# lambdaclass/lambda_elliptic_curves

Hardware: AMD Instinct MI355X
Metric: NTT elems/sec (Stark252 radix-2, 2^24, forward, bit-exact vs CPU: see 'bit_exact') [+ MSM G1 point-adds/sec under 'msm'] (higher is better)
Workload: dtype u32x8 (256-bit Montgomery, 32-bit limbs)

## Files before the change

### lambda_elliptic_curves_amd/csrc/field.cuh

```cuda
#pragma once
#include <stdint.h>

#if defined(__HIPCC__)
#include <hip/hip_runtime.h>
#define LW_HD __host__ __device__ __forceinline__
#else
#define LW_HD inline
#endif

namespace lw {

struct Stark252 {
    static constexpr int N = 8;
    static constexpr bool LAZY = true;
    static constexpr uint32_t INV = 0xffffffffu;
    static constexpr uint32_t TWO_ADICITY = 192;
    LW_HD static constexpr uint32_t p(int i) {
        constexpr uint32_t t[N] = {0x00000001u, 0x00000000u, 0x00000000u, 0x00000000u, 0x00000000u, 0x00000000u, 0x00000011u, 0x08000000u};
        return t[i];
    }
    LW_HD static constexpr uint32_t one(int i) {
        constexpr uint32_t t[N] = {0xffffffe1u, 0xffffffffu, 0xffffffffu, 0xffffffffu, 0xffffffffu, 0xffffffffu, 0xfffffdf0u, 0x07ffffffu};
        return t[i];
    }
// ... 231 lines not shown
#pragma unroll
    for (int i = 0; i < N; i++) {
        uint64_t c = 0;
#pragma unroll
        for (int j = 0; j < N; j++) {
            c += (uint64_t)a.v[j] * b.v[i] + t[j];
            t[j] = (uint32_t)c;
            c >>= 32;
        }
        uint32_t tN = (uint32_t)c;
        uint32_t m = t[0] * F::INV;
        c = ((uint64_t)m * F::p(0) + t[0]) >> 32;
#pragma unroll
        for (int j = 1; j < N; j++) {
            c += (uint64_t)m * F::p(j) + t[j];
            t[j - 1] = (uint32_t)c;
            c >>= 32;
        }
        c += tN;
        t[N - 1] = (uint32_t)c;
    }
    Fe<F> r;
#pragma unroll
    for (int i = 0; i < N; i++) r.v[i] = t[i];
    return reduce_once<F>(r);
}

#if !defined(__HIP_DEVICE_COMPILE__) && defined(__SIZEOF_INT128__)
#define LW_HOST_MUL64 1
template <class F>
inline Fe<F> fe_mul_host64(const Fe<F> &a, const Fe<F> &b) {
    constexpr int N = F::N, M = N / 2;
    static_assert(N % 2 == 0, "even number of 32-bit limbs");
    typedef unsigned __int128 u128;
    uint64_t A[M], B[M], P[M], t[M + 2];
    for (int i = 0; i < M; i++) {
        A[i] = (uint64_t)a.v[2 * i] | ((uint64_t)a.v[2 * i + 1] << 32);
        B[i] = (uint64_t)b.v[2 * i] | ((uint64_t)b.v[2 * i + 1] << 32);
        P[i] = (uint64_t)F::p(2 * i) | ((uint64_t)F::p(2 * i + 1) << 32);
    }
    for (int i = 0; i < M + 2; i++) t[i] = 0;
    uint64_t z = (uint64_t)(0u - F::INV);
    z *= 2 - P[0] * z;
    const uint64_t inv = 0 - z;
    for (int i = 0; i < M; i++) {
        u128 c = 0;
        for (int j = 0; j < M; j++) {
            c += (u128)A[j] * B[i] + t[j];
            t[j] = (uint64_t)c;
            c >>= 64;
        }
        c += t[M];
        t[M] = (uint64_t)c;
        t[M + 1] = (uint64_t)(c >> 64);
        const uint64_t m = t[0] * inv;
        c = ((u128)m * P[0] + t[0]) >> 64;
        for (int j = 1; j < M; j++) {
            c += (u128)m * P[j] + t[j];
            t[j - 1] = (uint64_t)c;
            c >>= 64;
        }
        c += t[M];
        t[M - 1] = (uint64_t)c;
        t[M] = t[M + 1] + (uint64_t)(c >> 64);
    }
    Fe<F> r;
    for (int i = 0; i < M; i++) {
        r.v[2 * i] = (uint32_t)t[i];
        r.v[2 * i + 1] = (uint32_t)(t[i] >> 32);
    }
    return reduce_once<F>(r);
}
#endif

#if defined(__HIP_DEVICE_COMPILE__)
#define LW_MAC_V(A, B) "v_mad_u64_u32 %0, vcc, " A ", " B ", %0\n\tv_addc_co_u32_e32 %1, vcc, 0, %1, vcc\n\t"

__device__ __forceinline__ void mac96_x1(uint64_t &lo, uint32_t &hi, uint32_t a0, uint32_t b0) {
    asm(LW_MAC_V("%2", "%3") : "+v"(lo), "+v"(hi) : "v"(a0), "v"(b0) : "vcc");
}
__device__ __forceinline__ void mac96_x2(uint64_t &lo, uint32_t &hi, uint32_t a0, uint32_t b0, uint32_t a1, uint32_t b1) {
    asm(LW_MAC_V("%2", "%3") LW_MAC_V("%4", "%5") : "+v"(lo), "+v"(hi) : "v"(a0), "v"(b0), "v"(a1), "v"(b1) : "vcc");
}
__device__ __forceinline__ void mac96_x4(uint64_t &lo, uint32_t &hi, uint32_t a0, uint32_t b0, uint32_t a1, uint32_t b1,
                                         uint32_t a2, uint32_t b2, uint32_t a3, uint32_t b3) {
    asm(LW_MAC_V("%2", "%3") LW_MAC_V("%4", "%5") LW_MAC_V("%6", "%7") LW_MAC_V("%8", "%9")
        : "+v"(lo), "+v"(hi)
        : "v"(a0), "v"(b0), "v"(a1), "v"(b1), "v"(a2), "v"(b2), "v"(a3), "v"(b3)
        : "vcc");
}
#define LW_MAC_FIRST(A, B, INIT) "v_mad_u64_u32 %0, vcc, " A ", " B ", " INIT "\n\tv_addc_co_u32_e64 %1, vcc, 0, 0, vcc\n\t"
__device__ __forceinline__ void mac96_first_x1(uint64_t &lo, uint32_t &hi, uint64_t init, uint32_t a0, uint32_t b0) {
    asm(LW_MAC_FIRST("%3", "%4", "%2") : "=v"(lo), "=v"(hi) : "v"(init), "v"(a0), "v"(b0) : "vcc");
}
__device__ __forceinline__ void mac96_first_x2(uint64_t &lo, uint32_t &hi, uint64_t init, uint32_t a0, uint32_t b0, uint32_t a1,
                                               uint32_t b1) {
    asm(LW_MAC_FIRST("%3", "%4", "%2") LW_MAC_V("%5", "%6")
        : "=&v"(lo), "=&v"(hi) : "v"(init), "v"(a0), "v"(b0), "v"(a1), "v"(b1) : "vcc");
}
__device__ __forceinline__ void mac96_first_x4(uint64_t &lo, uint32_t &hi, uint64_t init, uint32_t a0, uint32_t b0, uint32_t a1,
                                               uint32_t b1, uint32_t a2, uint32_t b2, uint32_t a3, uint32_t b3) {
    asm(LW_MAC_FIRST("%3", "%4", "%2") LW_MAC_V("%5", "%6") LW_MAC_V("%7", "%8") LW_MAC_V("%9", "%10")
        : "=&v"(lo), "=&v"(hi)
        : "v"(init), "v"(a0), "v"(b0), "v"(a1), "v"(b1), "v"(a2), "v"(b2), "v"(a3), "v"(b3)
        : "vcc");
}
template <uint32_t C>
__device__ __forceinline__ void mac96_c1(uint64_t &lo, uint32_t &hi, uint32_t m0) {
    if constexpr (C == 0) {
    } else if constexpr (C <= 64) {
        asm(LW_MAC_V("%2", "%3") : "+v"(lo), "+v"(hi) : "v"(m0), "n"(C) : "vcc");
    } else {
        asm(LW_MAC_V("%2", "%3") : "+v"(lo), "+v"(hi) : "v"(m0), "s"(C) : "vcc");
    }
}
template <uint32_t C0, uint32_t C1, uint32_t C2, uint32_t C3>
__device__ __forceinline__ void mac96_s4(uint64_t &lo, uint32_t &hi, uint32_t m0, uint32_t m1, uint32_t m2, uint32_t m3) {
    asm(LW_MAC_V("%2", "%3") LW_MAC_V("%4", "%5") LW_MAC_V("%6", "%7") LW_MAC_V("%8", "%9")
        : "+v"(lo), "+v"(hi)
        : "v"(m0), "s"(C0), "v"(m1), "s"(C1), "v"(m2), "s"(C2), "v"(m3), "s"(C3)
        : "vcc");
}

template <class F, int K, int I, int IEND>
__device__ __forceinline__ void col_ab(uint64_t &lo, uint32_t &hi, const Fe<F> &a, const Fe<F> &b) {
    if constexpr (I + 4 <= IEND) {
        mac96_x4(lo, hi, a.v[I], b.v[K - I], a.v[I + 1], b.v[K - I - 1], a.v[I + 2], b.v[K - I - 2], a.v[I + 3], b.v[K - I - 3]);
        col_ab<F, K, I + 4, IEND>(lo, hi, a, b);
    } else if constexpr (I + 2 <= IEND) {
        mac96_x2(lo, hi, a.v[I], b.v[K - I], a.v[I + 1], b.v[K - I - 1]);
        col_ab<F, K, I + 2, IEND>(lo, hi, a, b);
    } else if constexpr (I + 1 <= IEND) {
        mac96_x1(lo, hi, a.v[I], b.v[K - I]);
    }
}
template <uint32_t C>
constexpr bool lw_is_literal() { return C > 64; }
template <class F, int K, int I, int IEND>
__device__ __forceinline__ void col_mp(uint64_t &lo, uint32_t &hi, const uint32_t (&m)[F::N]) {
    if constexpr (I + 4 <= IEND) {
        if constexpr (lw_is_literal<F::p(K - I)>() && lw_is_literal<F::p(K - I - 1)>() && lw_is_literal<F::p(K - I - 2)>() &&
                      lw_is_literal<F::p(K - I - 3)>()) {
            mac96_s4<F::p(K - I), F::p(K - I - 1), F::p(K - I - 2), F::p(K - I - 3)>(lo, hi, m[I], m[I + 1], m[I + 2], m[I + 3]);
            col_mp<F, K, I + 4, IEND>(lo, hi, m);
        } else {
            mac96_c1<F::p(K - I)>(lo, hi, m[I]);
            col_mp<F, K, I + 1, IEND>(lo, hi, m);
        }
    } else if constexpr (I + 1 <= IEND) {
        mac96_c1<F::p(K - I)>(lo, hi, m[I]);
        col_mp<F, K, I + 1, IEND>(lo, hi, m);
    }
}
#include "mac_chains.inc"

template <class F, int LO, int HI>
constexpr bool lw_all_literal() {
    for (int i = LO; i < HI; i++)
        if (F::p(i) <= 64) return false;
    return true;
}

template <class F, int K, int I, int IEND>
__device__ __forceinline__ void col_ab_first(uint64_t &lo, uint32_t &hi, uint64_t init, const Fe<F> &a, const Fe<F> &b) {
    if constexpr (I + 4 <= IEND) {
        mac96_first_x4(lo, hi, init, a.v[I], b.v[K - I], a.v[I + 1], b.v[K - I - 1], a.v[I + 2], b.v[K - I - 2], a.v[I + 3], b.v[K - I - 3]);
        col_ab<F, K, I + 4, IEND>(lo, hi, a, b);
    } else if constexpr (I + 2 <= IEND) {
        mac96_first_x2(lo, hi, init, a.v[I], b.v[K - I], a.v[I + 1], b.v[K - I - 1]);
        col_ab<F, K, I + 2, IEND>(lo, hi, a, b);
    } else {
        static_assert(I + 1 <= IEND, "column without products");
        mac96_first_x1(lo, hi, init, a.v[I], b.v[K - I]);
    }
}
template <class F, int P, int K>
__device__ __forceinline__ void fips_col(uint64_t init, const Fe<F> *const (&a)[P], const Fe<F> *const (&b)[P], uint32_t (&m)[F::N],
                                         uint32_t (&t)[F::N]) {
    constexpr int N = F::N;
    if constexpr (K == 2 * N - 1) {
        t[N - 1] = (uint32_t)init;
    } else {
        uint64_t lo;
        uint32_t hi;
        if constexpr (K < N) {
#if defined(LW_NO_COLUMN_CHAINS)
            col_ab_first<F, K, 0, K + 1>(lo, hi, init, *a[0], *b[0]);
#else
            col_ab_first_dispatch<F, K, 0, K + 1>(lo, hi, init, *a[0], *b[0]);
#endif
            if constexpr (P > 1) col_ab<F, K, 0, K + 1>(lo, hi, *a[1], *b[1]);
            if constexpr (P > 2) col_ab<F, K, 0, K + 1>(lo, hi, *a[2], *b[2]);
            if constexpr (P > 3) col_ab<F, K, 0, K + 1>(lo, hi, *a[3], *b[3]);
#if defined(LW_NO_COLUMN_CHAINS)
            col_mp<F, K, 0, K>(lo, hi, m);
#else
            if constexpr (K >= 1 && lw_all_literal<F, 1, K + 1>()) col_mp_dispatch<F, K, 0, K>(lo, hi, m);
            else col_mp<F, K, 0, K>(lo, hi, m);
#endif
            uint32_t mk;
            if constexpr (F::INV == 0xffffffffu) mk = 0u - (uint32_t)lo;
            else mk = (uint32_t)lo * F::INV;
            m[K] = mk;
            mac96_c1<F::p(0)>(lo, hi, mk);
        } else {
#if defined(LW_NO_COLUMN_CHAINS)
            col_ab_first<F, K, K - N + 1, N>(lo, hi, init, *a[0], *b[0]);
#else
            col_ab_first_dispatch<F, K, K - N + 1, 2 * N - 1 - K>(lo, hi, init, *a[0], *b[0]);
#endif
            if constexpr (P > 1) col_ab<F, K, K - N + 1, N>(lo, hi, *a[1], *b[1]);
            if constexpr (P > 2) col_ab<F, K, K - N + 1, N>(lo, hi, *a[2], *b[2]);
            if constexpr (P > 3) col_ab<F, K, K - N + 1, N>(lo, hi, *a[3], *b[3]);
#if defined(LW_NO_COLUMN_CHAINS)
            col_mp<F, K, K - N + 1, N>(lo, hi, m);
#else
            if constexpr (lw_all_literal<F, K - N + 1, N>()) col_mp_dispatch<F, K, K - N + 1, 2 * N - 1 - K>(lo, hi, m);
            else col_mp<F, K, K - N + 1, N>(lo, hi, m);
#endif
            t[K - N] = (uint32_t)lo;
        }
        fips_col<F, P, K + 1>((lo >> 32) | ((uint64_t)hi << 32), a, b, m, t);
    }
}
template <class F>
__device__ __forceinline__ Fe<F> fe_mul_gfx9(const Fe<F> &a, const Fe<F> &b) {
    constexpr int N = F::N;
    uint32_t m[N], t[N];
    const Fe<F> *const pa[1] = {&a}, *const pb[1] = {&b};
    fips_col<F, 1, 0>(0ull, pa, pb, m, t);
    Fe<F> r;
#pragma unroll
    for (int i = 0; i < N; i++) r.v[i] = t[i];
    return reduce_once<F>(r);
}
#endif

template <class F>
LW_HD Fe<F> fe_mul(const Fe<F> &a, const Fe<F> &b) {
#if defined(__HIP_DEVICE_COMPILE__)
    return fe_mul_gfx9<F>(a, b);
#elif defined(LW_HOST_MUL64)
    return fe_mul_host64<F>(a, b);
#else
    return fe_mul_portable<F>(a, b);
#endif
}

template <class F>
LW_HD Fe<F> fe_sqr(const Fe<F> &a) { return fe_mul<F>(a, a); }

template <class F>
LW_HD Fe<F> fe_neg_raw(const Fe<F> &a) {
    uint32_t pk[F::N];
    limbs_kp<F, 0>(pk);
    Fe<F> r;
    limbs_sub<F::N>(r.v, pk, a.v);
    return r;
}
template <class F>
LW_HD Fe<F> fe_neg_raw_2p(const Fe<F> &a) {
    uint32_t pk[F::N];
    limbs_kp<F, 1>(pk);
    Fe<F> r;
    limbs_sub<F::N>(r.v, pk, a.v);
    return r;
}
template <class F, int P, int KSUM = P>
LW_HD Fe<F> fe_dot(const Fe<F> *const (&a)[P], const Fe<F> *const (&b)[P]) {
    static_assert(P >= 1 && P <= 4, "fe_dot: 1..4 products");
    static_assert(KSUM >= P, "fe_dot: KSUM counts every product at least once");
    static_assert((uint64_t)KSUM * ((uint64_t)F::p(F::N - 1) + 1) <= (1ull << 32), "fe_dot: sum of products would exceed 2p after reduction");
#if defined(__HIP_DEVICE_COMPILE__)
    constexpr int N = F::N;
    uint32_t m[N], t[N];
    fips_col<F, P, 0>(0ull, a, b, m, t);
    Fe<F> r;
#pragma unroll
    for (int i = 0; i < N; i++) r.v[i] = t[i];
    return reduce_once<F>(r);
#else
    static_assert(KSUM == P, "fe_dot: unreduced operands are a device-code feature");
    Fe<F> acc = fe_mul<F>(reduce_once<F>(*a[0]), *b[0]);
    for (int q = 1; q < P; q++) acc = fe_add<F>(acc, fe_mul<F>(reduce_once<F>(*a[q]), *b[q]));
    return acc;
#endif
}

template <class F, int LOGK>
LW_HD Fe<F> fe_cond_sub_kp(const Fe<F> &a) {
    constexpr int N = F::N;
    uint32_t kp[N];
    limbs_kp<F, LOGK>(kp);
    Fe<F> d;
    const uint32_t borrow = limbs_sub<N>(d.v, a.v, kp);
    Fe<F> r;
#pragma unroll
    for (int i = 0; i < N; i++) r.v[i] = borrow ? a.v[i] : d.v[i];
    return r;
}
LW_HD Fe<Stark252> fe_reduce_full(const Fe<Stark252> &x) {
    const uint32_t q = x.v[7] >> 27;
    const uint32_t z = lw_k(0u);
    const uint32_t sub[8] = {q, z, z, z, z, z, 17u * q, q << 27};
    Fe<Stark252> d;
    const uint32_t borrow = limbs_sub<8>(d.v, x.v, sub);
    uint32_t pm[8];
    limbs_p_masked<Stark252>(pm, 0u - borrow);
    Fe<Stark252> r;
    limbs_add<8>(r.v, d.v, pm);
    return r;
}
template <class F>
LW_HD Fe<F> fe_reduce_full(const Fe<F> &x) { return reduce_once<F>(x); }

template <class F>
LW_HD Fe<F> fe_add_raw(const Fe<F> &a, const Fe<F> &b) {
    Fe<F> s;
    limbs_add<F::N>(s.v, a.v, b.v);
    return s;
}
template <class F>
LW_HD Fe<F> fe_add2p_sub_raw(const Fe<F> &a, const Fe<F> &b) {
    constexpr int N = F::N;
    uint32_t kp[N];
    limbs_kp<F, 1>(kp);
    Fe<F> d, r;
    limbs_sub<N>(d.v, a.v, b.v);
    limbs_add<N>(r.v, d.v, kp);
    return r;
}
template <class F>
LW_HD Fe<F> fe_mul_lazy(const Fe<F> &a, const Fe<F> &b) {
#if defined(__HIP_DEVICE_COMPILE__)
    constexpr int N = F::N;
    uint32_t m[N], t[N];
    const Fe<F> *const pa[1] = {&a}, *const pb[1] = {&b};
    fips_col<F, 1, 0>(0ull, pa, pb, m, t);
    Fe<F> r;
#pragma unroll
    for (int i = 0; i < N; i++) r.v[i] = t[i];
    return r;
#else
    return fe_mul_portable<F>(a, b);
#endif
}

template <class F>
LW_HD Fe<F> fe_pow_u64(Fe<F> base, uint64_t e) {
    Fe<F> r = Fe<F>::one();
    while (e) {
        if (e & 1) r = fe_mul<F>(r, base);
        base = fe_sqr<F>(base);
        e >>= 1;
    }
    return r;
}

template <class F>
LW_HD Fe<F> fe_inv(const Fe<F> &a) {
    constexpr int N = F::N;
    uint32_t e[N];
    uint64_t borrow = 2;
#pragma unroll
    for (int i = 0; i < N; i++) {
        uint64_t t = (uint64_t)F::p(i) - borrow;
        e[i] = (uint32_t)t;
        borrow = (t >> 32) & 1;
    }
    Fe<F> r = Fe<F>::one();
    for (int i = N - 1; i >= 0; i--) {
        for (int bit = 31; bit >= 0; bit--) {
            r = fe_sqr<F>(r);
            if ((e[i] >> bit) & 1) r = fe_mul<F>(r, a);
        }
    }
    return r;
}

template <class F>
LW_HD constexpr int fe_modulus_bits() {
    int top = 0;
    for (int b = 0; b < 32; b++)
        if ((F::p(F::N - 1) >> b) & 1u) top = b + 1;
    return 32 * (F::N - 1) + top;
}
template <int N>
LW_HD uint32_t bingcd_update_ab(uint32_t (&x)[N], uint32_t (&y)[N], int32_t f, int32_t g, int32_t h, int32_t k) {
    int64_t cx = 0, cy = 0;
    uint32_t wx[N + 1], wy[N + 1];
#pragma unroll
    for (int i = 0; i < N; i++) {
        const int64_t zx = (int64_t)x[i] * f + (int64_t)y[i] * g + cx;
        const int64_t zy = (int64_t)x[i] * h + (int64_t)y[i] * k + cy;
        wx[i] = (uint32_t)zx;
        wy[i] = (uint32_t)zy;
        cx = zx >> 32;
        cy = zy >> 32;
    }
    wx[N] = (uint32_t)cx;
    wy[N] = (uint32_t)cy;
    const uint32_t nx = (uint32_t)((uint64_t)cx >> 63), ny = (uint32_t)((uint64_t)cy >> 63);
    uint32_t carx = nx, cary = ny;
#pragma unroll
    for (int i = 0; i < N; i++) {
        uint32_t rx = (wx[i] >> 30) | (wx[i + 1] << 2), ry = (wy[i] >> 30) | (wy[i + 1] << 2);
        rx ^= 0u - nx;
        ry ^= 0u - ny;
        const uint32_t sx = rx + carx, sy = ry + cary;
        carx = sx < rx ? 1u : 0u;
        cary = sy < ry ? 1u : 0u;
        x[i] = sx;
        y[i] = sy;
    }
    return nx | (ny << 1);
}
template <class F>
LW_HD void bingcd_update_uv(uint32_t (&u)[F::N], uint32_t (&v)[F::N], int32_t f, int32_t g, int32_t h, int32_t k) {
    constexpr int N = F::N;
    const uint32_t fu = ((uint32_t)(u[0] * (uint32_t)f + v[0] * (uint32_t)g) * F::INV) & 0x3fffffffu;
    const uint32_t fv = ((uint32_t)(u[0] * (uint32_t)h + v[0] * (uint32_t)k) * F::INV) & 0x3fffffffu;
    int64_t cu = 0, cv = 0;
    uint32_t wu[N + 1], wv[N + 1];
#pragma unroll
    for (int i = 0; i < N; i++) {
        const int64_t zu = (int64_t)u[i] * f + (int64_t)v[i] * g + (int64_t)((uint64_t)F::p(i) * fu) + cu;
        const int64_t zv = (int64_t)u[i] * h + (int64_t)v[i] * k + (int64_t)((uint64_t)F::p(i) * fv) + cv;
        wu[i] = (uint32_t)zu;
        wv[i] = (uint32_t)zv;
        cu = zu >> 32;
        cv = zv >> 32;
    }
    wu[N] = (uint32_t)cu;
    wv[N] = (uint32_t)cv;
    const uint32_t nu = (uint32_t)((uint64_t)cu >> 63), nv = (uint32_t)((uint64_t)cv >> 63);
    uint32_t ru[N], rv[N];
#pragma unroll
    for (int i = 0; i < N; i++) {
        ru[i] = (wu[i] >> 30) | (wu[i + 1] << 2);
        rv[i] = (wv[i] >> 30) | (wv[i + 1] << 2);
    }
    uint32_t pk[N], du[N], dv[N], su[N], sv[N];
#pragma unroll
    for (int i = 0; i < N; i++) pk[i] = F::p(i);
    const uint32_t bu = limbs_sub<N>(du, ru, pk), bv = limbs_sub<N>(dv, rv, pk);
    limbs_add<N>(su, ru, pk);
    limbs_add<N>(sv, rv, pk);
#pragma unroll
    for (int i = 0; i < N; i++) {
        u[i] = nu ? su[i] : (bu ? ru[i] : du[i]);
        v[i] = nv ? sv[i] : (bv ? rv[i] : dv[i]);
    }
}
template <class F>
LW_HD Fe<F> fe_inv_int_bingcd(const Fe<F> &y) {
    constexpr int N = F::N;
    constexpr int ROUNDS = (2 * fe_modulus_bits<F>()) / 29 + 2;
    uint32_t a[N], b[N], u[N], v[N];
#pragma unroll
    for (int i = 0; i < N; i++) {
        a[i] = y.v[i];
        b[i] = F::p(i);
        u[i] = i == 0 ? 1u : 0u;
        v[i] = 0u;
    }
#pragma nounroll
    for (int round = 0; round < ROUNDS; round++) {
        uint32_t a0 = 0, a1 = 0, b0 = 0, b1 = 0, c0 = 0xffffffffu, c1 = 0xffffffffu;
#pragma unroll
        for (int j = N - 1; j >= 0; j--) {
            const uint32_t aw = a[j], bw = b[j];
            a0 ^= (a0 ^ aw) & c0;
            a1 ^= (a1 ^ aw) & c1;
            b0 ^= (b0 ^ bw) & c0;
            b1 ^= (b1 ^ bw) & c1;
            c1 = c0;
            c0 &= ((aw | bw) == 0u) ? 0xffffffffu : 0u;
        }
        a1 |= a0 & c1;
        a0 &= ~c1;
        b1 |= b0 & c1;
        b0 &= ~c1;
        uint64_t a_hi = ((uint64_t)a0 << 32) | a1, b_hi = ((uint64_t)b0 << 32) | b1;
        uint32_t a_lo = a[0], b_lo = b[0];
        int32_t pa = 1, pb = 0, qa = 0, qb = 1;
#pragma unroll 2
        for (int i = 0; i < 30; i++) {
            const uint32_t r = a_hi > b_hi ? 1u : 0u;
            const uint32_t oa = (a_lo >> i) & 1u, ob = (b_lo >> i) & 1u;
            const uint32_t cAB = oa & ob & r, cBA = oa & ob & (r ^ 1u), cA = cAB | (oa ^ 1u);
            const uint32_t mAB = 0u - cAB, mBA = 0u - cBA, mA = 0u - cA;
// ... 118 lines not shown
```

### lambda_elliptic_curves_amd/csrc/mac_chains.inc

```

template <class F, int K, int I>
__device__ __forceinline__ void col_ab_first_n1(uint64_t &lo, uint32_t &hi, uint64_t init, const Fe<F> &a, const Fe<F> &b) {
    asm(LW_MAC_FIRST("%3", "%4", "%2")
        : "=v"(lo), "=v"(hi)
        : "v"(init), "v"(a.v[I + 0]), "v"(b.v[K - I - 0])
        : "vcc");
}

template <class F, int K, int I>
__device__ __forceinline__ void col_ab_first_n2(uint64_t &lo, uint32_t &hi, uint64_t init, const Fe<F> &a, const Fe<F> &b) {
    asm(LW_MAC_FIRST("%3", "%4", "%2") LW_MAC_V("%5", "%6")
        : "=&v"(lo), "=&v"(hi)
        : "v"(init), "v"(a.v[I + 0]), "v"(b.v[K - I - 0]), "v"(a.v[I + 1]), "v"(b.v[K - I - 1])
        : "vcc");
}

template <class F, int K, int I>
__device__ __forceinline__ void col_ab_first_n3(uint64_t &lo, uint32_t &hi, uint64_t init, const Fe<F> &a, const Fe<F> &b) {
    asm(LW_MAC_FIRST("%3", "%4", "%2") LW_MAC_V("%5", "%6") LW_MAC_V("%7", "%8")
        : "=&v"(lo), "=&v"(hi)
        : "v"(init), "v"(a.v[I + 0]), "v"(b.v[K - I - 0]), "v"(a.v[I + 1]), "v"(b.v[K - I - 1]), "v"(a.v[I + 2]), "v"(b.v[K - I - 2])
        : "vcc");
}

// ... 39 lines not shown

template <class F, int K, int I>
__device__ __forceinline__ void col_ab_first_n9(uint64_t &lo, uint32_t &hi, uint64_t init, const Fe<F> &a, const Fe<F> &b) {
    asm(LW_MAC_FIRST("%3", "%4", "%2") LW_MAC_V("%5", "%6") LW_MAC_V("%7", "%8") LW_MAC_V("%9", "%10") LW_MAC_V("%11", "%12") LW_MAC_V("%13", "%14") LW_MAC_V("%15", "%16") LW_MAC_V("%17", "%18") LW_MAC_V("%19", "%20")
        : "=&v"(lo), "=&v"(hi)
        : "v"(init), "v"(a.v[I + 0]), "v"(b.v[K - I - 0]), "v"(a.v[I + 1]), "v"(b.v[K - I - 1]), "v"(a.v[I + 2]), "v"(b.v[K - I - 2]), "v"(a.v[I + 3]), "v"(b.v[K - I - 3]), "v"(a.v[I + 4]), "v"(b.v[K - I - 4]), "v"(a.v[I + 5]), "v"(b.v[K - I - 5]), "v"(a.v[I + 6]), "v"(b.v[K - I - 6]), "v"(a.v[I + 7]), "v"(b.v[K - I - 7]), "v"(a.v[I + 8]), "v"(b.v[K - I - 8])
        : "vcc");
}

template <class F, int K, int I>
__device__ __forceinline__ void col_ab_first_n10(uint64_t &lo, uint32_t &hi, uint64_t init, const Fe<F> &a, const Fe<F> &b) {
    asm(LW_MAC_FIRST("%3", "%4", "%2") LW_MAC_V("%5", "%6") LW_MAC_V("%7", "%8") LW_MAC_V("%9", "%10") LW_MAC_V("%11", "%12") LW_MAC_V("%13", "%14") LW_MAC_V("%15", "%16") LW_MAC_V("%17", "%18") LW_MAC_V("%19", "%20") LW_MAC_V("%21", "%22")
        : "=&v"(lo), "=&v"(hi)
        : "v"(init), "v"(a.v[I + 0]), "v"(b.v[K - I - 0]), "v"(a.v[I + 1]), "v"(b.v[K - I - 1]), "v"(a.v[I + 2]), "v"(b.v[K - I - 2]), "v"(a.v[I + 3]), "v"(b.v[K - I - 3]), "v"(a.v[I + 4]), "v"(b.v[K - I - 4]), "v"(a.v[I + 5]), "v"(b.v[K - I - 5]), "v"(a.v[I + 6]), "v"(b.v[K - I - 6]), "v"(a.v[I + 7]), "v"(b.v[K - I - 7]), "v"(a.v[I + 8]), "v"(b.v[K - I - 8]), "v"(a.v[I + 9]), "v"(b.v[K - I - 9])
        : "vcc");
}

template <class F, int K, int I>
__device__ __forceinline__ void col_ab_first_n11(uint64_t &lo, uint32_t &hi, uint64_t init, const Fe<F> &a, const Fe<F> &b) {
    asm(LW_MAC_FIRST("%3", "%4", "%2") LW_MAC_V("%5", "%6") LW_MAC_V("%7", "%8") LW_MAC_V("%9", "%10") LW_MAC_V("%11", "%12") LW_MAC_V("%13", "%14") LW_MAC_V("%15", "%16") LW_MAC_V("%17", "%18") LW_MAC_V("%19", "%20") LW_MAC_V("%21", "%22") LW_MAC_V("%23", "%24")
        : "=&v"(lo), "=&v"(hi)
        : "v"(init), "v"(a.v[I + 0]), "v"(b.v[K - I - 0]), "v"(a.v[I + 1]), "v"(b.v[K - I - 1]), "v"(a.v[I + 2]), "v"(b.v[K - I - 2]), "v"(a.v[I + 3]), "v"(b.v[K - I - 3]), "v"(a.v[I + 4]), "v"(b.v[K - I - 4]), "v"(a.v[I + 5]), "v"(b.v[K - I - 5]), "v"(a.v[I + 6]), "v"(b.v[K - I - 6]), "v"(a.v[I + 7]), "v"(b.v[K - I - 7]), "v"(a.v[I + 8]), "v"(b.v[K - I - 8]), "v"(a.v[I + 9]), "v"(b.v[K - I - 9]), "v"(a.v[I + 10]), "v"(b.v[K - I - 10])
        : "vcc");
}

template <class F, int K, int I>
__device__ __forceinline__ void col_ab_first_n12(uint64_t &lo, uint32_t &hi, uint64_t init, const Fe<F> &a, const Fe<F> &b) {
    asm(LW_MAC_FIRST("%3", "%4", "%2") LW_MAC_V("%5", "%6") LW_MAC_V("%7", "%8") LW_MAC_V("%9", "%10") LW_MAC_V("%11", "%12") LW_MAC_V("%13", "%14") LW_MAC_V("%15", "%16") LW_MAC_V("%17", "%18") LW_MAC_V("%19", "%20") LW_MAC_V("%21", "%22") LW_MAC_V("%23", "%24") LW_MAC_V("%25", "%26")
        : "=&v"(lo), "=&v"(hi)
        : "v"(init), "v"(a.v[I + 0]), "v"(b.v[K - I - 0]), "v"(a.v[I + 1]), "v"(b.v[K - I - 1]), "v"(a.v[I + 2]), "v"(b.v[K - I - 2]), "v"(a.v[I + 3]), "v"(b.v[K - I - 3]), "v"(a.v[I + 4]), "v"(b.v[K - I - 4]), "v"(a.v[I + 5]), "v"(b.v[K - I - 5]), "v"(a.v[I + 6]), "v"(b.v[K - I - 6]), "v"(a.v[I + 7]), "v"(b.v[K - I - 7]), "v"(a.v[I + 8]), "v"(b.v[K - I - 8]), "v"(a.v[I + 9]), "v"(b.v[K - I - 9]), "v"(a.v[I + 10]), "v"(b.v[K - I - 10]), "v"(a.v[I + 11]), "v"(b.v[K - I - 11])
        : "vcc");
}

template <class F, int K, int I>
__device__ __forceinline__ void col_mp_n1(uint64_t &lo, uint32_t &hi, const uint32_t (&m)[F::N]) {
    asm(LW_MAC_V("%2", "%3")
        : "+v"(lo), "+v"(hi)
        : "v"(m[I + 0]), "s"(F::p(K - I - 0))
        : "vcc");
}

template <class F, int K, int I>
__device__ __forceinline__ void col_mp_n2(uint64_t &lo, uint32_t &hi, const uint32_t (&m)[F::N]) {
    asm(LW_MAC_V("%2", "%3") LW_MAC_V("%4", "%5")
        : "+v"(lo), "+v"(hi)
        : "v"(m[I + 0]), "s"(F::p(K - I - 0)), "v"(m[I + 1]), "s"(F::p(K - I - 1))
        : "vcc");
}

template <class F, int K, int I>
__device__ __forceinline__ void col_mp_n3(uint64_t &lo, uint32_t &hi, const uint32_t (&m)[F::N]) {
    asm(LW_MAC_V("%2", "%3") LW_MAC_V("%4", "%5") LW_MAC_V("%6", "%7")
        : "+v"(lo), "+v"(hi)
        : "v"(m[I + 0]), "s"(F::p(K - I - 0)), "v"(m[I + 1]), "s"(F::p(K - I - 1)), "v"(m[I + 2]), "s"(F::p(K - I - 2))
        : "vcc");
}

template <class F, int K, int I>
__device__ __forceinline__ void col_mp_n4(uint64_t &lo, uint32_t &hi, const uint32_t (&m)[F::N]) {
    asm(LW_MAC_V("%2", "%3") LW_MAC_V("%4", "%5") LW_MAC_V("%6", "%7") LW_MAC_V("%8", "%9")
        : "+v"(lo), "+v"(hi)
        : "v"(m[I + 0]), "s"(F::p(K - I - 0)), "v"(m[I + 1]), "s"(F::p(K - I - 1)), "v"(m[I + 2]), "s"(F::p(K - I - 2)), "v"(m[I + 3]), "s"(F::p(K - I - 3))
        : "vcc");
}

template <class F, int K, int I>
__device__ __forceinline__ void col_mp_n5(uint64_t &lo, uint32_t &hi, const uint32_t (&m)[F::N]) {
    asm(LW_MAC_V("%2", "%3") LW_MAC_V("%4", "%5") LW_MAC_V("%6", "%7") LW_MAC_V("%8", "%9") LW_MAC_V("%10", "%11")
        : "+v"(lo), "+v"(hi)
        : "v"(m[I + 0]), "s"(F::p(K - I - 0)), "v"(m[I + 1]), "s"(F::p(K - I - 1)), "v"(m[I + 2]), "s"(F::p(K - I - 2)), "v"(m[I + 3]), "s"(F::p(K - I - 3)), "v"(m[I + 4]), "s"(F::p(K - I - 4))
        : "vcc");
}

template <class F, int K, int I>
__device__ __forceinline__ void col_mp_n6(uint64_t &lo, uint32_t &hi, const uint32_t (&m)[F::N]) {
    asm(LW_MAC_V("%2", "%3") LW_MAC_V("%4", "%5") LW_MAC_V("%6", "%7") LW_MAC_V("%8", "%9") LW_MAC_V("%10", "%11") LW_MAC_V("%12", "%13")
        : "+v"(lo), "+v"(hi)
        : "v"(m[I + 0]), "s"(F::p(K - I - 0)), "v"(m[I + 1]), "s"(F::p(K - I - 1)), "v"(m[I + 2]), "s"(F::p(K - I - 2)), "v"(m[I + 3]), "s"(F::p(K - I - 3)), "v"(m[I + 4]), "s"(F::p(K - I - 4)), "v"(m[I + 5]), "s"(F::p(K - I - 5))
        : "vcc");
}

template <class F, int K, int I>
__device__ __forceinline__ void col_mp_n7(uint64_t &lo, uint32_t &hi, const uint32_t (&m)[F::N]) {
    asm(LW_MAC_V("%2", "%3") LW_MAC_V("%4", "%5") LW_MAC_V("%6", "%7") LW_MAC_V("%8", "%9") LW_MAC_V("%10", "%11") LW_MAC_V("%12", "%13") LW_MAC_V("%14", "%15")
        : "+v"(lo), "+v"(hi)
        : "v"(m[I + 0]), "s"(F::p(K - I - 0)), "v"(m[I + 1]), "s"(F::p(K - I - 1)), "v"(m[I + 2]), "s"(F::p(K - I - 2)), "v"(m[I + 3]), "s"(F::p(K - I - 3)), "v"(m[I + 4]), "s"(F::p(K - I - 4)), "v"(m[I + 5]), "s"(F::p(K - I - 5)), "v"(m[I + 6]), "s"(F::p(K - I - 6))
        : "vcc");
}

template <class F, int K, int I>
__device__ __forceinline__ void col_mp_n8(uint64_t &lo, uint32_t &hi, const uint32_t (&m)[F::N]) {
    asm(LW_MAC_V("%2", "%3") LW_MAC_V("%4", "%5") LW_MAC_V("%6", "%7") LW_MAC_V("%8", "%9") LW_MAC_V("%10", "%11") LW_MAC_V("%12", "%13") LW_MAC_V("%14", "%15") LW_MAC_V("%16", "%17")
        : "+v"(lo), "+v"(hi)
        : "v"(m[I + 0]), "s"(F::p(K - I - 0)), "v"(m[I + 1]), "s"(F::p(K - I - 1)), "v"(m[I + 2]), "s"(F::p(K - I - 2)), "v"(m[I + 3]), "s"(F::p(K - I - 3)), "v"(m[I + 4]), "s"(F::p(K - I - 4)), "v"(m[I + 5]), "s"(F::p(K - I - 5)), "v"(m[I + 6]), "s"(F::p(K - I - 6)), "v"(m[I + 7]), "s"(F::p(K - I - 7))
        : "vcc");
}

template <class F, int K, int I>
__device__ __forceinline__ void col_mp_n9(uint64_t &lo, uint32_t &hi, const uint32_t (&m)[F::N]) {
    asm(LW_MAC_V("%2", "%3") LW_MAC_V("%4", "%5") LW_MAC_V("%6", "%7") LW_MAC_V("%8", "%9") LW_MAC_V("%10", "%11") LW_MAC_V("%12", "%13") LW_MAC_V("%14", "%15") LW_MAC_V("%16", "%17") LW_MAC_V("%18", "%19")
        : "+v"(lo), "+v"(hi)
        : "v"(m[I + 0]), "s"(F::p(K - I - 0)), "v"(m[I + 1]), "s"(F::p(K - I - 1)), "v"(m[I + 2]), "s"(F::p(K - I - 2)), "v"(m[I + 3]), "s"(F::p(K - I - 3)), "v"(m[I + 4]), "s"(F::p(K - I - 4)), "v"(m[I + 5]), "s"(F::p(K - I - 5)), "v"(m[I + 6]), "s"(F::p(K - I - 6)), "v"(m[I + 7]), "s"(F::p(K - I - 7)), "v"(m[I + 8]), "s"(F::p(K - I - 8))
        : "vcc");
}

template <class F, int K, int I>
__device__ __forceinline__ void col_mp_n10(uint64_t &lo, uint32_t &hi, const uint32_t (&m)[F::N]) {
    asm(LW_MAC_V("%2", "%3") LW_MAC_V("%4", "%5") LW_MAC_V("%6", "%7") LW_MAC_V("%8", "%9") LW_MAC_V("%10", "%11") LW_MAC_V("%12", "%13") LW_MAC_V("%14", "%15") LW_MAC_V("%16", "%17") LW_MAC_V("%18", "%19") LW_MAC_V("%20", "%21")
        : "+v"(lo), "+v"(hi)
        : "v"(m[I + 0]), "s"(F::p(K - I - 0)), "v"(m[I + 1]), "s"(F::p(K - I - 1)), "v"(m[I + 2]), "s"(F::p(K - I - 2)), "v"(m[I + 3]), "s"(F::p(K - I - 3)), "v"(m[I + 4]), "s"(F::p(K - I - 4)), "v"(m[I + 5]), "s"(F::p(K - I - 5)), "v"(m[I + 6]), "s"(F::p(K - I - 6)), "v"(m[I + 7]), "s"(F::p(K - I - 7)), "v"(m[I + 8]), "s"(F::p(K - I - 8)), "v"(m[I + 9]), "s"(F::p(K - I - 9))
        : "vcc");
}

template <class F, int K, int I>
__device__ __forceinline__ void col_mp_n11(uint64_t &lo, uint32_t &hi, const uint32_t (&m)[F::N]) {
    asm(LW_MAC_V("%2", "%3") LW_MAC_V("%4", "%5") LW_MAC_V("%6", "%7") LW_MAC_V("%8", "%9") LW_MAC_V("%10", "%11") LW_MAC_V("%12", "%13") LW_MAC_V("%14", "%15") LW_MAC_V("%16", "%17") LW_MAC_V("%18", "%19") LW_MAC_V("%20", "%21") LW_MAC_V("%22", "%23")
        : "+v"(lo), "+v"(hi)
        : "v"(m[I + 0]), "s"(F::p(K - I - 0)), "v"(m[I + 1]), "s"(F::p(K - I - 1)), "v"(m[I + 2]), "s"(F::p(K - I - 2)), "v"(m[I + 3]), "s"(F::p(K - I - 3)), "v"(m[I + 4]), "s"(F::p(K - I - 4)), "v"(m[I + 5]), "s"(F::p(K - I - 5)), "v"(m[I + 6]), "s"(F::p(K - I - 6)), "v"(m[I + 7]), "s"(F::p(K - I - 7)), "v"(m[I + 8]), "s"(F::p(K - I - 8)), "v"(m[I + 9]), "s"(F::p(K - I - 9)), "v"(m[I + 10]), "s"(F::p(K - I - 10))
        : "vcc");
}

template <class F, int K, int I, int CNT>
__device__ __forceinline__ void col_ab_first_dispatch(uint64_t &lo, uint32_t &hi, uint64_t init, const Fe<F> &a, const Fe<F> &b) {
    if constexpr (CNT == 1) col_ab_first_n1<F, K, I>(lo, hi, init, a, b);
    else if constexpr (CNT == 2) col_ab_first_n2<F, K, I>(lo, hi, init, a, b);
    else if constexpr (CNT == 3) col_ab_first_n3<F, K, I>(lo, hi, init, a, b);
    else if constexpr (CNT == 4) col_ab_first_n4<F, K, I>(lo, hi, init, a, b);
    else if constexpr (CNT == 5) col_ab_first_n5<F, K, I>(lo, hi, init, a, b);
    else if constexpr (CNT == 6) col_ab_first_n6<F, K, I>(lo, hi, init, a, b);
    else if constexpr (CNT == 7) col_ab_first_n7<F, K, I>(lo, hi, init, a, b);
    else if constexpr (CNT == 8) col_ab_first_n8<F, K, I>(lo, hi, init, a, b);
    else if constexpr (CNT == 9) col_ab_first_n9<F, K, I>(lo, hi, init, a, b);
    else if constexpr (CNT == 10) col_ab_first_n10<F, K, I>(lo, hi, init, a, b);
    else if constexpr (CNT == 11) col_ab_first_n11<F, K, I>(lo, hi, init, a, b);
    else if constexpr (CNT == 12) col_ab_first_n12<F, K, I>(lo, hi, init, a, b);
    else static_assert(CNT >= 1 && CNT <= 12, "unsupported MAC count");
}

template <class F, int K, int I, int CNT>
__device__ __forceinline__ void col_mp_dispatch(uint64_t &lo, uint32_t &hi, const uint32_t (&m)[F::N]) {
    if constexpr (CNT == 1) col_mp_n1<F, K, I>(lo, hi, m);
    else if constexpr (CNT == 2) col_mp_n2<F, K, I>(lo, hi, m);
    else if constexpr (CNT == 3) col_mp_n3<F, K, I>(lo, hi, m);
    else if constexpr (CNT == 4) col_mp_n4<F, K, I>(lo, hi, m);
    else if constexpr (CNT == 5) col_mp_n5<F, K, I>(lo, hi, m);
    else if constexpr (CNT == 6) col_mp_n6<F, K, I>(lo, hi, m);
    else if constexpr (CNT == 7) col_mp_n7<F, K, I>(lo, hi, m);
    else if constexpr (CNT == 8) col_mp_n8<F, K, I>(lo, hi, m);
    else if constexpr (CNT == 9) col_mp_n9<F, K, I>(lo, hi, m);
    else if constexpr (CNT == 10) col_mp_n10<F, K, I>(lo, hi, m);
    else if constexpr (CNT == 11) col_mp_n11<F, K, I>(lo, hi, m);
    else static_assert(CNT >= 1 && CNT <= 11, "unsupported MAC count");
}
```

Measured before the change: 12.42 billion.

## Fuse Stark252 Montgomery product columns with unit-limb reduction in hand-written asm

```diff
diff --git a/lambda_elliptic_curves_amd/csrc/field.cuh b/lambda_elliptic_curves_amd/csrc/field.cuh
--- a/lambda_elliptic_curves_amd/csrc/field.cuh
+++ b/lambda_elliptic_curves_amd/csrc/field.cuh
@@ -407,6 +407,12 @@
         col_mp<F, K, I + 1, IEND>(lo, hi, m);
     }
 }
+template <class F>
+struct lw_fused_columns {
+    static constexpr bool value = false;
+};
+template <class F, int K>
+struct FusedCol;
 #include "mac_chains.inc"
 
 template <class F, int LO, int HI>
@@ -478,12 +484,58 @@
         fips_col<F, P, K + 1>((lo >> 32) | ((uint64_t)hi << 32), a, b, m, t);
     }
 }
+__device__ __forceinline__ void lw_redc_unit(uint32_t &m, uint32_t &mid, uint32_t &top, uint32_t t, uint32_t w1, uint32_t w2) {
+    asm("v_sub_co_u32_e32 %0, vcc, 0, %3\n\t"
+        "v_addc_co_u32_e32 %1, vcc, 0, %4, vcc\n\t"
+        "v_addc_co_u32_e32 %2, vcc, 0, %5, vcc"
+        : "=&v"(m), "=&v"(mid), "=v"(top)
+        : "v"(t), "v"(w1), "v"(w2)
+        : "vcc");
+}
+__device__ __forceinline__ void lw_redc_unit0(uint32_t &m, uint32_t &mid, uint32_t &top, uint32_t t, uint32_t w1) {
+    asm("v_sub_co_u32_e32 %0, vcc, 0, %3\n\t"
+        "v_addc_co_u32_e32 %1, vcc, 0, %4, vcc\n\t"
+        "v_addc_co_u32_e64 %2, vcc, 0, 0, vcc"
+        : "=&v"(m), "=&v"(mid), "=v"(top)
+        : "v"(t), "v"(w1)
+        : "vcc");
+}
+template <class F, int K>
+__device__ __forceinline__ void fips_fused(uint64_t init, const Fe<F> &a, const Fe<F> &b, uint32_t (&m)[F::N], uint32_t (&t)[F::N]) {
+    constexpr int N = F::N;
+    static_assert(F::p(0) == 1u && F::INV == 0xffffffffu, "fused columns need a unit low limb of the modulus");
+    if constexpr (K == 2 * N - 1) {
+        t[N - 1] = (uint32_t)init;
+    } else {
+        uint64_t lo;
+        uint32_t hi;
+        FusedCol<F, K>::run(lo, hi, init, a, b, m);
+        if constexpr (K < N) {
+            uint32_t mid, top;
+            if constexpr (K == 0) lw_redc_unit0(m[0], mid, top, (uint32_t)lo, (uint32_t)(lo >> 32));
+            else lw_redc_unit(m[K], mid, top, (uint32_t)lo, (uint32_t)(lo >> 32), hi);
+            fips_fused<F, K + 1>(((uint64_t)top << 32) | mid, a, b, m, t);
+        } else {
+            t[K - N] = (uint32_t)lo;
+            fips_fused<F, K + 1>((lo >> 32) | ((uint64_t)hi << 32), a, b, m, t);
+        }
+    }
+}
+template <class F>
+__device__ __forceinline__ void fips_product(const Fe<F> &a, const Fe<F> &b, uint32_t (&t)[F::N]) {
+    uint32_t m[F::N];
+    if constexpr (lw_fused_columns<F>::value) {
+        fips_fused<F, 0>(0ull, a, b, m, t);
+    } else {
+        const Fe<F> *const pa[1] = {&a}, *const pb[1] = {&b};
+        fips_col<F, 1, 0>(0ull, pa, pb, m, t);
+    }
+}
 template <class F>
 __device__ __forceinline__ Fe<F> fe_mul_gfx9(const Fe<F> &a, const Fe<F> &b) {
     constexpr int N = F::N;
-    uint32_t m[N], t[N];
-    const Fe<F> *const pa[1] = {&a}, *const pb[1] = {&b};
-    fips_col<F, 1, 0>(0ull, pa, pb, m, t);
+    uint32_t t[N];
+    fips_product<F>(a, b, t);
     Fe<F> r;
 #pragma unroll
     for (int i = 0; i < N; i++) r.v[i] = t[i];
@@ -589,9 +641,8 @@
 LW_HD Fe<F> fe_mul_lazy(const Fe<F> &a, const Fe<F> &b) {
 #if defined(__HIP_DEVICE_COMPILE__)
     constexpr int N = F::N;
-    uint32_t m[N], t[N];
-    const Fe<F> *const pa[1] = {&a}, *const pb[1] = {&b};
-    fips_col<F, 1, 0>(0ull, pa, pb, m, t);
+    uint32_t t[N];
+    fips_product<F>(a, b, t);
     Fe<F> r;
 #pragma unroll
     for (int i = 0; i < N; i++) r.v[i] = t[i];
diff --git a/lambda_elliptic_curves_amd/csrc/mac_chains.inc b/lambda_elliptic_curves_amd/csrc/mac_chains.inc
--- a/lambda_elliptic_curves_amd/csrc/mac_chains.inc
+++ b/lambda_elliptic_curves_amd/csrc/mac_chains.inc
@@ -215,3 +215,288 @@
     else if constexpr (CNT == 11) col_mp_n11<F, K, I>(lo, hi, m);
     else static_assert(CNT >= 1 && CNT <= 11, "unsupported MAC count");
 }
+
+static_assert(Stark252::N == 8 && Stark252::p(0) == 0x00000001u && Stark252::p(1) == 0x00000000u && Stark252::p(2) == 0x00000000u && Stark252::p(3) == 0x00000000u && Stark252::p(4) == 0x00000000u && Stark252::p(5) == 0x00000000u && Stark252::p(6) == 0x00000011u && Stark252::p(7) == 0x08000000u, "modulus changed: rerun tools/gen_mac_chains.py");
+template <>
+struct lw_fused_columns<Stark252> {
+    static constexpr bool value = true;
+};
+
+template <>
+struct FusedCol<Stark252, 0> {
+    __device__ static __forceinline__ void run(uint64_t &lo, uint32_t &hi, uint64_t init, const Fe<Stark252> &a, const Fe<Stark252> &b, const uint32_t (&m)[8]) {
+        asm("v_mad_u64_u32 %0, vcc, %1, %2, 0\n\t"
+            : "=v"(lo)
+            : "v"(a.v[0]), "v"(b.v[0])
+            : "vcc");
+        hi = 0;
+    }
+};
+
+template <>
+struct FusedCol<Stark252, 1> {
+    __device__ static __forceinline__ void run(uint64_t &lo, uint32_t &hi, uint64_t init, const Fe<Stark252> &a, const Fe<Stark252> &b, const uint32_t (&m)[8]) {
+        asm("v_mad_u64_u32 %0, vcc, %3, %4, %2\n\t"
+            "v_addc_co_u32_e64 %1, vcc, 0, 0, vcc\n\t"
+            "v_mad_u64_u32 %0, vcc, %5, %6, %0\n\t"
+            "v_addc_co_u32_e32 %1, vcc, 0, %1, vcc\n\t"
+            : "=&v"(lo), "=&v"(hi)
+            : "v"(init), "v"(a.v[0]), "v"(b.v[1]), "v"(a.v[1]), "v"(b.v[0])
+            : "vcc");
+    }
+};
+
+template <>
+struct FusedCol<Stark252, 2> {
+    __device__ static __forceinline__ void run(uint64_t &lo, uint32_t &hi, uint64_t init, const Fe<Stark252> &a, const Fe<Stark252> &b, const uint32_t (&m)[8]) {
+        asm("v_mad_u64_u32 %0, vcc, %3, %4, %2\n\t"
+            "v_addc_co_u32_e64 %1, vcc, 0, 0, vcc\n\t"
+            "v_mad_u64_u32 %0, vcc, %5, %6, %0\n\t"
+            "v_addc_co_u32_e32 %1, vcc, 0, %1, vcc\n\t"
+            "v_mad_u64_u32 %0, vcc, %7, %8, %0\n\t"
+            "v_addc_co_u32_e32 %1, vcc, 0, %1, vcc\n\t"
+            : "=&v"(lo), "=&v"(hi)
+            : "v"(init), "v"(a.v[0]), "v"(b.v[2]), "v"(a.v[1]), "v"(b.v[1]), "v"(a.v[2]), "v"(b.v[0])
+            : "vcc");
+    }
+};
+
+template <>
+struct FusedCol<Stark252, 3> {
+    __device__ static __forceinline__ void run(uint64_t &lo, uint32_t &hi, uint64_t init, const Fe<Stark252> &a, const Fe<Stark252> &b, const uint32_t (&m)[8]) {
+        asm("v_mad_u64_u32 %0, vcc, %3, %4, %2\n\t"
+            "v_addc_co_u32_e64 %1, vcc, 0, 0, vcc\n\t"
+            "v_mad_u64_u32 %0, vcc, %5, %6, %0\n\t"
+            "v_addc_co_u32_e32 %1, vcc, 0, %1, vcc\n\t"
+            "v_mad_u64_u32 %0, vcc, %7, %8, %0\n\t"
+            "v_addc_co_u32_e32 %1, vcc, 0, %1, vcc\n\t"
+            "v_mad_u64_u32 %0, vcc, %9, %10, %0\n\t"
+            "v_addc_co_u32_e32 %1, vcc, 0, %1, vcc\n\t"
+            : "=&v"(lo), "=&v"(hi)
+            : "v"(init), "v"(a.v[0]), "v"(b.v[3]), "v"(a.v[1]), "v"(b.v[2]), "v"(a.v[2]), "v"(b.v[1]), "v"(a.v[3]), "v"(b.v[0])
+            : "vcc");
+    }
+};
+
+template <>
+struct FusedCol<Stark252, 4> {
+    __device__ static __forceinline__ void run(uint64_t &lo, uint32_t &hi, uint64_t init, const Fe<Stark252> &a, const Fe<Stark252> &b, const uint32_t (&m)[8]) {
+        asm("v_mad_u64_u32 %0, vcc, %3, %4, %2\n\t"
+            "v_addc_co_u32_e64 %1, vcc, 0, 0, vcc\n\t"
+            "v_mad_u64_u32 %0, vcc, %5, %6, %0\n\t"
+            "v_addc_co_u32_e32 %1, vcc, 0, %1, vcc\n\t"
+            "v_mad_u64_u32 %0, vcc, %7, %8, %0\n\t"
+            "v_addc_co_u32_e32 %1, vcc, 0, %1, vcc\n\t"
+            "v_mad_u64_u32 %0, vcc, %9, %10, %0\n\t"
+            "v_addc_co_u32_e32 %1, vcc, 0, %1, vcc\n\t"
+            "v_mad_u64_u32 %0, vcc, %11, %12, %0\n\t"
+            "v_addc_co_u32_e32 %1, vcc, 0, %1, vcc\n\t"
+            : "=&v"(lo), "=&v"(hi)
+            : "v"(init), "v"(a.v[0]), "v"(b.v[4]), "v"(a.v[1]), "v"(b.v[3]), "v"(a.v[2]), "v"(b.v[2]), "v"(a.v[3]), "v"(b.v[1]), "v"(a.v[4]), "v"(b.v[0])
+            : "vcc");
+    }
+};
+
+template <>
+struct FusedCol<Stark252, 5> {
+    __device__ static __forceinline__ void run(uint64_t &lo, uint32_t &hi, uint64_t init, const Fe<Stark252> &a, const Fe<Stark252> &b, const uint32_t (&m)[8]) {
+        asm("v_mad_u64_u32 %0, vcc, %3, %4, %2\n\t"
+            "v_addc_co_u32_e64 %1, vcc, 0, 0, vcc\n\t"
+            "v_mad_u64_u32 %0, vcc, %5, %6, %0\n\t"
+            "v_addc_co_u32_e32 %1, vcc, 0, %1, vcc\n\t"
+            "v_mad_u64_u32 %0, vcc, %7, %8, %0\n\t"
+            "v_addc_co_u32_e32 %1, vcc, 0, %1, vcc\n\t"
+            "v_mad_u64_u32 %0, vcc, %9, %10, %0\n\t"
+            "v_addc_co_u32_e32 %1, vcc, 0, %1, vcc\n\t"
+            "v_mad_u64_u32 %0, vcc, %11, %12, %0\n\t"
+            "v_addc_co_u32_e32 %1, vcc, 0, %1, vcc\n\t"
+            "v_mad_u64_u32 %0, vcc, %13, %14, %0\n\t"
+            "v_addc_co_u32_e32 %1, vcc, 0, %1, vcc\n\t"
+            : "=&v"(lo), "=&v"(hi)
+            : "v"(init), "v"(a.v[0]), "v"(b.v[5]), "v"(a.v[1]), "v"(b.v[4]), "v"(a.v[2]), "v"(b.v[3]), "v"(a.v[3]), "v"(b.v[2]), "v"(a.v[4]), "v"(b.v[1]), "v"(a.v[5]), "v"(b.v[0])
+            : "vcc");
+    }
+};
+
+template <>
+struct FusedCol<Stark252, 6> {
+    __device__ static __forceinline__ void run(uint64_t &lo, uint32_t &hi, uint64_t init, const Fe<Stark252> &a, const Fe<Stark252> &b, const uint32_t (&m)[8]) {
+        asm("v_mad_u64_u32 %0, vcc, %3, 17, %2\n\t"
+            "v_mad_u64_u32 %0, vcc, %4, %5, %0\n\t"
+            "v_addc_co_u32_e64 %1, vcc, 0, 0, vcc\n\t"
+            "v_mad_u64_u32 %0, vcc, %6, %7, %0\n\t"
+            "v_addc_co_u32_e32 %1, vcc, 0, %1, vcc\n\t"
+            "v_mad_u64_u32 %0, vcc, %8, %9, %0\n\t"
+            "v_addc_co_u32_e32 %1, vcc, 0, %1, vcc\n\t"
+            "v_mad_u64_u32 %0, vcc, %10, %11, %0\n\t"
+            "v_addc_co_u32_e32 %1, vcc, 0, %1, vcc\n\t"
+            "v_mad_u64_u32 %0, vcc, %12, %13, %0\n\t"
+            "v_addc_co_u32_e32 %1, vcc, 0, %1, vcc\n\t"
+            "v_mad_u64_u32 %0, vcc, %14, %15, %0\n\t"
+            "v_addc_co_u32_e32 %1, vcc, 0, %1, vcc\n\t"
+            "v_mad_u64_u32 %0, vcc, %16, %17, %0\n\t"
+            "v_addc_co_u32_e32 %1, vcc, 0, %1, vcc\n\t"
+            : "=&v"(lo), "=&v"(hi)
+            : "v"(init), "v"(m[0]), "v"(a.v[0]), "v"(b.v[6]), "v"(a.v[1]), "v"(b.v[5]), "v"(a.v[2]), "v"(b.v[4]), "v"(a.v[3]), "v"(b.v[3]), "v"(a.v[4]), "v"(b.v[2]), "v"(a.v[5]), "v"(b.v[1]), "v"(a.v[6]), "v"(b.v[0])
+            : "vcc");
+    }
+};
+
+template <>
+struct FusedCol<Stark252, 7> {
+    __device__ static __forceinline__ void run(uint64_t &lo, uint32_t &hi, uint64_t init, const Fe<Stark252> &a, const Fe<Stark252> &b, const uint32_t (&m)[8]) {
+        asm("v_mad_u64_u32 %0, vcc, %3, %4, %2\n\t"
+            "v_mad_u64_u32 %0, vcc, %5, 17, %0\n\t"
+            "v_mad_u64_u32 %0, vcc, %6, %7, %0\n\t"
+            "v_addc_co_u32_e64 %1, vcc, 0, 0, vcc\n\t"
+            "v_mad_u64_u32 %0, vcc, %8, %9, %0\n\t"
+            "v_addc_co_u32_e32 %1, vcc, 0, %1, vcc\n\t"
+            "v_mad_u64_u32 %0, vcc, %10, %11, %0\n\t"
+            "v_addc_co_u32_e32 %1, vcc, 0, %1, vcc\n\t"
+            "v_mad_u64_u32 %0, vcc, %12, %13, %0\n\t"
+            "v_addc_co_u32_e32 %1, vcc, 0, %1, vcc\n\t"
+            "v_mad_u64_u32 %0, vcc, %14, %15, %0\n\t"
+            "v_addc_co_u32_e32 %1, vcc, 0, %1, vcc\n\t"
+            "v_mad_u64_u32 %0, vcc, %16, %17, %0\n\t"
+            "v_addc_co_u32_e32 %1, vcc, 0, %1, vcc\n\t"
+            "v_mad_u64_u32 %0, vcc, %18, %19, %0\n\t"
+            "v_addc_co_u32_e32 %1, vcc, 0, %1, vcc\n\t"
+            "v_mad_u64_u32 %0, vcc, %20, %21, %0\n\t"
+            "v_addc_co_u32_e32 %1, vcc, 0, %1, vcc\n\t"
+            : "=&v"(lo), "=&v"(hi)
+            : "v"(init), "v"(m[0]), "s"(Stark252::p(7)), "v"(m[1]), "v"(a.v[0]), "v"(b.v[7]), "v"(a.v[1]), "v"(b.v[6]), "v"(a.v[2]), "v"(b.v[5]), "v"(a.v[3]), "v"(b.v[4]), "v"(a.v[4]), "v"(b.v[3]), "v"(a.v[5]), "v"(b.v[2]), "v"(a.v[6]), "v"(b.v[1]), "v"(a.v[7]), "v"(b.v[0])
+            : "vcc");
+    }
+};
+
+template <>
+struct FusedCol<Stark252, 8> {
+    __device__ static __forceinline__ void run(uint64_t &lo, uint32_t &hi, uint64_t init, const Fe<Stark252> &a, const Fe<Stark252> &b, const uint32_t (&m)[8]) {
+        asm("v_mad_u64_u32 %0, vcc, %3, %4, %2\n\t"
+            "v_mad_u64_u32 %0, vcc, %5, 17, %0\n\t"
+            "v_mad_u64_u32 %0, vcc, %6, %7, %0\n\t"
+            "v_addc_co_u32_e64 %1, vcc, 0, 0, vcc\n\t"
+            "v_mad_u64_u32 %0, vcc, %8, %9, %0\n\t"
+            "v_addc_co_u32_e32 %1, vcc, 0, %1, vcc\n\t"
+            "v_mad_u64_u32 %0, vcc, %10, %11, %0\n\t"
+            "v_addc_co_u32_e32 %1, vcc, 0, %1, vcc\n\t"
+            "v_mad_u64_u32 %0, vcc, %12, %13, %0\n\t"
+            "v_addc_co_u32_e32 %1, vcc, 0, %1, vcc\n\t"
+            "v_mad_u64_u32 %0, vcc, %14, %15, %0\n\t"
+            "v_addc_co_u32_e32 %1, vcc, 0, %1, vcc\n\t"
+            "v_mad_u64_u32 %0, vcc, %16, %17, %0\n\t"
+            "v_addc_co_u32_e32 %1, vcc, 0, %1, vcc\n\t"
+            "v_mad_u64_u32 %0, vcc, %18, %19, %0\n\t"
+            "v_addc_co_u32_e32 %1, vcc, 0, %1, vcc\n\t"
+            : "=&v"(lo), "=&v"(hi)
+            : "v"(init), "v"(m[1]), "s"(Stark252::p(7)), "v"(m[2]), "v"(a.v[1]), "v"(b.v[7]), "v"(a.v[2]), "v"(b.v[6]), "v"(a.v[3]), "v"(b.v[5]), "v"(a.v[4]), "v"(b.v[4]), "v"(a.v[5]), "v"(b.v[3]), "v"(a.v[6]), "v"(b.v[2]), "v"(a.v[7]), "v"(b.v[1])
+            : "vcc");
+    }
+};
+
+template <>
+struct FusedCol<Stark252, 9> {
+    __device__ static __forceinline__ void run(uint64_t &lo, uint32_t &hi, uint64_t init, const Fe<Stark252> &a, const Fe<Stark252> &b, const uint32_t (&m)[8]) {
+        asm("v_mad_u64_u32 %0, vcc, %3, %4, %2\n\t"
+            "v_mad_u64_u32 %0, vcc, %5, 17, %0\n\t"
+            "v_mad_u64_u32 %0, vcc, %6, %7, %0\n\t"
+            "v_addc_co_u32_e64 %1, vcc, 0, 0, vcc\n\t"
+            "v_mad_u64_u32 %0, vcc, %8, %9, %0\n\t"
+            "v_addc_co_u32_e32 %1, vcc, 0, %1, vcc\n\t"
+            "v_mad_u64_u32 %0, vcc, %10, %11, %0\n\t"
+            "v_addc_co_u32_e32 %1, vcc, 0, %1, vcc\n\t"
+            "v_mad_u64_u32 %0, vcc, %12, %13, %0\n\t"
+            "v_addc_co_u32_e32 %1, vcc, 0, %1, vcc\n\t"
+            "v_mad_u64_u32 %0, vcc, %14, %15, %0\n\t"
+            "v_addc_co_u32_e32 %1, vcc, 0, %1, vcc\n\t"
+            "v_mad_u64_u32 %0, vcc, %16, %17, %0\n\t"
+            "v_addc_co_u32_e32 %1, vcc, 0, %1, vcc\n\t"
+            : "=&v"(lo), "=&v"(hi)
+            : "v"(init), "v"(m[2]), "s"(Stark252::p(7)), "v"(m[3]), "v"(a.v[2]), "v"(b.v[7]), "v"(a.v[3]), "v"(b.v[6]), "v"(a.v[4]), "v"(b.v[5]), "v"(a.v[5]), "v"(b.v[4]), "v"(a.v[6]), "v"(b.v[3]), "v"(a.v[7]), "v"(b.v[2])
+            : "vcc");
+    }
+};
+
+template <>
+struct FusedCol<Stark252, 10> {
+    __device__ static __forceinline__ void run(uint64_t &lo, uint32_t &hi, uint64_t init, const Fe<Stark252> &a, const Fe<Stark252> &b, const uint32_t (&m)[8]) {
+        asm("v_mad_u64_u32 %0, vcc, %3, %4, %2\n\t"
+            "v_mad_u64_u32 %0, vcc, %5, 17, %0\n\t"
+            "v_mad_u64_u32 %0, vcc, %6, %7, %0\n\t"
+            "v_addc_co_u32_e64 %1, vcc, 0, 0, vcc\n\t"
+            "v_mad_u64_u32 %0, vcc, %8, %9, %0\n\t"
+            "v_addc_co_u32_e32 %1, vcc, 0, %1, vcc\n\t"
+            "v_mad_u64_u32 %0, vcc, %10, %11, %0\n\t"
+            "v_addc_co_u32_e32 %1, vcc, 0, %1, vcc\n\t"
+            "v_mad_u64_u32 %0, vcc, %12, %13, %0\n\t"
+            "v_addc_co_u32_e32 %1, vcc, 0, %1, vcc\n\t"
+            "v_mad_u64_u32 %0, vcc, %14, %15, %0\n\t"
+            "v_addc_co_u32_e32 %1, vcc, 0, %1, vcc\n\t"
+            : "=&v"(lo), "=&v"(hi)
+            : "v"(init), "v"(m[3]), "s"(Stark252::p(7)), "v"(m[4]), "v"(a.v[3]), "v"(b.v[7]), "v"(a.v[4]), "v"(b.v[6]), "v"(a.v[5]), "v"(b.v[5]), "v"(a.v[6]), "v"(b.v[4]), "v"(a.v[7]), "v"(b.v[3])
+            : "vcc");
+    }
+};
+
+template <>
+struct FusedCol<Stark252, 11> {
+    __device__ static __forceinline__ void run(uint64_t &lo, uint32_t &hi, uint64_t init, const Fe<Stark252> &a, const Fe<Stark252> &b, const uint32_t (&m)[8]) {
+        asm("v_mad_u64_u32 %0, vcc, %3, %4, %2\n\t"
+            "v_mad_u64_u32 %0, vcc, %5, 17, %0\n\t"
+            "v_mad_u64_u32 %0, vcc, %6, %7, %0\n\t"
+            "v_addc_co_u32_e64 %1, vcc, 0, 0, vcc\n\t"
+            "v_mad_u64_u32 %0, vcc, %8, %9, %0\n\t"
+            "v_addc_co_u32_e32 %1, vcc, 0, %1, vcc\n\t"
+            "v_mad_u64_u32 %0, vcc, %10, %11, %0\n\t"
+            "v_addc_co_u32_e32 %1, vcc, 0, %1, vcc\n\t"
+            "v_mad_u64_u32 %0, vcc, %12, %13, %0\n\t"
+            "v_addc_co_u32_e32 %1, vcc, 0, %1, vcc\n\t"
+            : "=&v"(lo), "=&v"(hi)
+            : "v"(init), "v"(m[4]), "s"(Stark252::p(7)), "v"(m[5]), "v"(a.v[4]), "v"(b.v[7]), "v"(a.v[5]), "v"(b.v[6]), "v"(a.v[6]), "v"(b.v[5]), "v"(a.v[7]), "v"(b.v[4])
+            : "vcc");
+    }
+};
+
+template <>
+struct FusedCol<Stark252, 12> {
+    __device__ static __forceinline__ void run(uint64_t &lo, uint32_t &hi, uint64_t init, const Fe<Stark252> &a, const Fe<Stark252> &b, const uint32_t (&m)[8]) {
+        asm("v_mad_u64_u32 %0, vcc, %3, %4, %2\n\t"
+            "v_mad_u64_u32 %0, vcc, %5, 17, %0\n\t"
+            "v_mad_u64_u32 %0, vcc, %6, %7, %0\n\t"
+            "v_addc_co_u32_e64 %1, vcc, 0, 0, vcc\n\t"
+            "v_mad_u64_u32 %0, vcc, %8, %9, %0\n\t"
+            "v_addc_co_u32_e32 %1, vcc, 0, %1, vcc\n\t"
+            "v_mad_u64_u32 %0, vcc, %10, %11, %0\n\t"
+            "v_addc_co_u32_e32 %1, vcc, 0, %1, vcc\n\t"
+            : "=&v"(lo), "=&v"(hi)
+            : "v"(init), "v"(m[5]), "s"(Stark252::p(7)), "v"(m[6]), "v"(a.v[5]), "v"(b.v[7]), "v"(a.v[6]), "v"(b.v[6]), "v"(a.v[7]), "v"(b.v[5])
+            : "vcc");
+    }
+};
+
+template <>
+struct FusedCol<Stark252, 13> {
+    __device__ static __forceinline__ void run(uint64_t &lo, uint32_t &hi, uint64_t init, const Fe<Stark252> &a, const Fe<Stark252> &b, const uint32_t (&m)[8]) {
+        asm("v_mad_u64_u32 %0, vcc, %3, %4, %2\n\t"
+            "v_mad_u64_u32 %0, vcc, %5, 17, %0\n\t"
+            "v_mad_u64_u32 %0, vcc, %6, %7, %0\n\t"
+            "v_addc_co_u32_e64 %1, vcc, 0, 0, vcc\n\t"
+            "v_mad_u64_u32 %0, vcc, %8, %9, %0\n\t"
+            "v_addc_co_u32_e32 %1, vcc, 0, %1, vcc\n\t"
+            : "=&v"(lo), "=&v"(hi)
+            : "v"(init), "v"(m[6]), "s"(Stark252::p(7)), "v"(m[7]), "v"(a.v[6]), "v"(b.v[7]), "v"(a.v[7]), "v"(b.v[6])
+            : "vcc");
+    }
+};
+
+template <>
+struct FusedCol<Stark252, 14> {
+    __device__ static __forceinline__ void run(uint64_t &lo, uint32_t &hi, uint64_t init, const Fe<Stark252> &a, const Fe<Stark252> &b, const uint32_t (&m)[8]) {
+        asm("v_mad_u64_u32 %0, vcc, %2, %3, %1\n\t"
+            "v_mad_u64_u32 %0, vcc, %4, %5, %0\n\t"
+            : "=&v"(lo)
+            : "v"(init), "v"(m[7]), "s"(Stark252::p(7)), "v"(a.v[7]), "v"(b.v[7])
+            : "vcc");
+        hi = 0;
+    }
+};
```

Measured after the change: 13.12 billion, median of 6. +5.6%, better.
